# ClickHouse/libhdfs3

Hardware: AMD Instinct MI355X
Metric: device-resident CRC32C GiB/s over 512 B HDFS chunks; % of HBM roofline (higher is better)
Workload: dtype u8

## Files before the change

### libhdfs3_amd/csrc/crc32c_device.h

```cpp
#pragma once
#include <hip/hip_ext.h>

#include <type_traits>

#include "crc32c_kernels.h"
#include "crc32c_tables.h"

namespace hdfs3crc {
namespace {

constexpr int kCopies = 32;
constexpr int kLdsBytes = 128 * 1024;
constexpr int kLdsSlots = kLdsBytes / 16;

typedef uint32_t u32x4 __attribute__((ext_vector_type(4)));

constexpr int kFillPerThread = kLdsSlots / kBlockThreads;

__device__ __forceinline__ void fetch_tables(uint32_t (&v)[kFillPerThread],
                                             const uint32_t *__restrict__ g_tab) {
#pragma unroll
    for (int i = 0; i < kFillPerThread; ++i) {
        const int s = i * kBlockThreads + threadIdx.x;
        const int rowset = s >> 12, entry = (s >> 4) & 255, half = (s >> 3) & 1;
// ... 426 lines not shown
constexpr int kFoldLdsOff = kLdsBytes;
constexpr int kLdsBytesWave = kLdsBytes + 32 * 1024;

struct NibFold {
    const uint8_t *f;
    __device__ __forceinline__ explicit NibFold(const uint32_t *lds)
        : f(reinterpret_cast<const uint8_t *>(lds) + kFoldLdsOff + 4 * (threadIdx.x & 63)) {}
    __device__ __forceinline__ uint32_t ld(uint32_t off) const {
        return *reinterpret_cast<const uint32_t *>(f + off);
    }
    __device__ __forceinline__ uint32_t apply(uint32_t x) const {
        const uint32_t a0 = ld(((x << 8) & 0xF00u) + 0 * 4096);
        const uint32_t a1 = ld(((x << 4) & 0xF00u) + 1 * 4096);
        const uint32_t a2 = ld((x & 0xF00u) + 2 * 4096);
        const uint32_t a3 = ld(((x >> 4) & 0xF00u) + 3 * 4096);
        const uint32_t a4 = ld(((x >> 8) & 0xF00u) + 4 * 4096);
        const uint32_t a5 = ld(((x >> 12) & 0xF00u) + 5 * 4096);
        const uint32_t a6 = ld(((x >> 16) & 0xF00u) + 6 * 4096);
        const uint32_t a7 = ld(((x >> 20) & 0xF00u) + 7 * 4096);
        return xor3(xor3(a0, a1, a2), xor3(a3, a4, a5), a6 ^ a7);
    }
};

struct Look {
    uint32_t v[4];
};
__device__ __forceinline__ Look lookups(const Lut &t, uint32_t x) {
    Look l;
    l.v[0] = t.at<0>(3, x);
    l.v[1] = t.at<1>(2, x);
    l.v[2] = t.at<2>(1, x);
    l.v[3] = t.at<3>(0, x);
    return l;
}
__device__ __forceinline__ uint32_t combine(const Look &l, uint32_t next) {
    return xor3(xor3(l.v[0], l.v[1], l.v[2]), l.v[3], next);
}

constexpr int kHalfFoldOff = kLdsBytes;

template <int OFF = kHalfFoldOff>
__device__ __forceinline__ uint32_t fold_half(const uint8_t *lds, uint32_t x) {
    const uint32_t lo = x & 0x0F0F0F0Fu, hi = (x >> 4) & 0x0F0F0F0Fu;
    const uint32_t fb = (OFF & ~0xFFFF) + 4 * (threadIdx.x & 31);
    auto at = [&](uint32_t src, uint32_t byte, int off) {
        const uint32_t addr = __builtin_amdgcn_perm(src, fb, 0x0C020000u | ((4u + byte) << 8));
        return *reinterpret_cast<const uint32_t *>(lds + addr + (OFF & 0xFFFF) + off);
    };
    const uint32_t a0 = at(lo, 0, 0), a1 = at(hi, 0, 128), a2 = at(lo, 1, 4096), a3 = at(hi, 1, 4096 + 128);
    const uint32_t a4 = at(lo, 2, 8192), a5 = at(hi, 2, 8192 + 128), a6 = at(lo, 3, 12288);
    const uint32_t a7 = at(hi, 3, 12288 + 128);
    return xor3(xor3(a0, a1, a2), xor3(a3, a4, a5), a6 ^ a7);
}


struct SegLaunch {
    const DevSegment *seg;
    uint32_t nseg;
    uint64_t units;
    uint64_t uniform;
    unsigned long long *result;
    int check_short_tail;
    uint64_t stride;
    uint32_t kq, kr;
    uint8_t *dense_words;
    const uint32_t *unit_seg;
    DevSegment inl[kInlineSegments];
};

template <bool VERIFY>
__global__ __launch_bounds__(kBlockThreads) void crc32c_packets_kernel(
    const uint8_t *arena_c, uint8_t *arena_w, const DevPacket *__restrict__ pk,
    uint64_t n, uint32_t bpc, int check_short_tail, unsigned long long *result,
    const uint32_t *__restrict__ g_tab) {
    __shared__ __attribute__((aligned(16))) uint32_t lds[kLdsBytes / 4];
    fill_tables(lds, g_tab);
    lds_barrier();
    const Lut t(lds);
    const uint32_t lane = threadIdx.x & 63;
    const uint64_t waves = uint64_t(gridDim.x) * (kBlockThreads / 64);
    for (uint64_t w = uint64_t(blockIdx.x) * (kBlockThreads / 64) + (threadIdx.x >> 6); w < n;
         w += waves) {
        const DevPacket d = pk[w];
        const uint32_t chunks = (d.data_len + bpc - 1) / bpc;
        const uint8_t *data = arena_c + d.data_off;
        const bool al4 = (reinterpret_cast<uintptr_t>(arena_c + d.crc_off) & 3u) == 0;
        for (uint32_t k = lane; k < chunks; k += 64) {
            const uint32_t off = k * bpc;
            const uint32_t sz = d.data_len - off < bpc ? d.data_len - off : bpc;
            const uint32_t c = ~crc_run_any(t, 0xFFFFFFFFu, data + off, sz);
            if constexpr (VERIFY) {
                if ((sz == bpc || check_short_tail) &&
                    load_be32(arena_c + d.crc_off + 4ull * k, al4) != c)
                    atomicMax(result, ~((uint64_t(w) << 32) | k));
            } else {
                store_be32(arena_w + d.crc_off + 4ull * k, c, al4);
            }
        }
    }
}


#if HDFS3_LAB
__device__ unsigned long long *g_lab_clk = nullptr;
__device__ unsigned int g_lab_clk_cap = 0;
__device__ unsigned int g_lab_clk_n = 0;
// ... 143 lines not shown
```

### libhdfs3_amd/csrc/crc32c_experiments.hip

```cpp
#include "crc32c_wave.h"

namespace hdfs3crc {
namespace {

template <int BPC, bool V>
hipError_t launch_exp(const LaunchEnv &env, int variant, const ChunkLaunch &a) {
    const auto [tab, fold, grid_cap, s] = std::tie(env.tables, env.fold, env.grid_cap, env.stream);
    if constexpr (BPC > kRoundBytes) {
        if (variant == 115) return launch_r3<BPC, V, 1, true, true>(a, tab, fold, grid_cap, s);
        if (variant == 123) return launch_r3<BPC, V, 1, true>(a, tab, fold, grid_cap, s);
    }
    if constexpr (BPC <= kRoundBytes) {
        switch (variant) {
        case 92:
            return launch_wave3<BPC, V, false, true, kLabEarly>(a, tab, fold, grid_cap, s);
        case 93:
            return launch_wave3<BPC, V, false, false>(a, tab, fold, grid_cap, s);
        case 94:
            return launch_wave3<BPC, V, false, V>(a, tab, fold, grid_cap, s);
        case 95:
            return launch_wave3<BPC, V, false, true, kLabNoHold>(a, tab, fold, grid_cap, s);
        case 77:
            return launch_wave3<BPC, V, false, true, kLabNoMath>(a, tab, fold, grid_cap, s);
        case 99:
        case 100: {
            const uint64_t units = a.len / kRoundBytes;
            const uint64_t npk = variant == 99 ? 1 : 8;
            const uint64_t upp = units / npk;
            if (a.len % kRoundBytes || units % npk || (upp & (upp - 1)) || a.chunk_base) return hipErrorInvalidValue;
            ChunkLaunch p = a;
            p.npk = npk;
            p.pitch = upp * kRoundBytes;
            p.crc_pitch = upp * (kRoundBytes / BPC) * 4;
            p.last_len = uint32_t(upp * kRoundBytes);
            if (!packet_geom(p.pitch, p.last_len, npk, BPC, &p.geom)) return hipErrorInvalidValue;
            return launch_wave3<BPC, V, true, false>(p, tab, fold, grid_cap, s);
        }
        case 115:
            return launch_wave3<BPC, V, false, true, kLabPrio>(a, tab, fold, grid_cap, s);
        case 117:
            return launch_wave3<BPC, V, false, true, kLabNoPrio>(a, tab, fold, grid_cap, s);
        case 118:
            return launch_wave3<BPC, V, false, true, kLabNoStore>(a, tab, fold, grid_cap, s);
        case 119:
            return launch_wave3<BPC, V, false, true, kLabNearStore>(a, tab, fold, grid_cap, s);
        case 123:
            return launch_wave3<BPC, V, false, true>(a, tab, fold, grid_cap, s);
        case 122:
            return launch_wave3<BPC, V, false, true, kLabNoStage>(a, tab, fold, grid_cap, s);
        case 130:
            return launch_wave3<BPC, V, false, true, kLabStageWin>(a, tab, fold, grid_cap, s);
        case 157:
            return launch_wave3<BPC, V, false, true, kLabFull16>(a, tab, fold, grid_cap, s);
        case 128:
            return launch_wave3<BPC, V, false, true, kLabStorePlain>(a, tab, fold, grid_cap, s);
        case 146:
            return launch_wave3<BPC, V, false, true, kLabClock | kLabMid>(a, tab, fold, grid_cap, s);
        case 147:
            return launch_wave3<BPC, V, false, true, kLabNoTabLoad | kLabClock | kLabMid>(a, tab, fold, grid_cap, s);
        case 148:
            return launch_wave3<BPC, V, false, true, kLabNoTabLoad>(a, tab, fold, grid_cap, s);
        case 137:
            return launch_wave3<BPC, V, false, true, kLabWg1024>(a, tab, fold, grid_cap, s);
        case 162:
            return launch_wave3<BPC, V, false, true, kLabOneRound>(a, tab, fold, grid_cap, s);
        case 132:
            return launch_wave3<BPC, V, false, true, 0, 256>(a, tab, fold, grid_cap, s);
        case 134:
            return launch_wave3<BPC, V, false, true, 0, 512>(a, tab, fold, grid_cap, s);
        case 125:
            return launch_wave3<BPC, V, false, true, kLabClock>(a, tab, fold, grid_cap, s);
        case 78:
            return launch_wave3<BPC, V, false, true, kLabNoMath | kLabNoFill>(a, tab, fold, grid_cap, s);
        default: return hipErrorInvalidValue;
        }
    }
    return hipErrorInvalidValue;
}

}

hipError_t launch_experiment(const LaunchEnv &env, int variant, const ChunkLaunch &a, bool verify) {
    return dispatch_bpc<true>(a.bpc, [&](auto bpc) {
        return verify ? launch_exp<bpc(), true>(env, variant, a) : launch_exp<bpc(), false>(env, variant, a);
    });
}

void set_variant(int v) { g_variant = v; }

hipError_t lab_clock_buffer(unsigned long long *d, unsigned int cap, unsigned int *n_out) {
    unsigned int n = 0;
    hipError_t e = hipMemcpyFromSymbol(&n, HIP_SYMBOL(g_lab_clk_n), sizeof n);
    if (e != hipSuccess) return e;
    if (n_out) *n_out = n;
    const unsigned int zero = 0;
    if ((e = hipMemcpyToSymbol(HIP_SYMBOL(g_lab_clk), &d, sizeof d)) != hipSuccess) return e;
    if ((e = hipMemcpyToSymbol(HIP_SYMBOL(g_lab_clk_cap), &cap, sizeof cap)) != hipSuccess) return e;
    return hipMemcpyToSymbol(HIP_SYMBOL(g_lab_clk_n), &zero, sizeof zero);
}

hipError_t lab_wave_buffer(unsigned long long *d, unsigned int cap, unsigned int *n_out) {
    if (n_out) *n_out = g_lab_seq.exchange(0);
    hipError_t e;
    const unsigned long long *none = nullptr;
    if ((e = hipMemcpyToSymbol(HIP_SYMBOL(g_lab_wave), &none, sizeof none)) != hipSuccess) return e;
    if (!d || !cap) return hipSuccess;
// ... 47 lines not shown
```

### libhdfs3_amd/csrc/crc32c_kernels.hip

```cpp
#include "crc32c_wave.h"

namespace hdfs3crc {

#if HDFS3_LAB
int g_variant = 0;
#endif

namespace {

inline int clamped_grid(uint64_t want, uint64_t cap) { return int(want < cap ? want : cap); }

template <int BPC, bool V>
hipError_t launch_r(const LaunchEnv &env, const ChunkLaunch &a) {
#if HDFS3_LAB
    if (g_variant != 0) return launch_experiment(env, g_variant, a, V);
#endif
    if constexpr (BPC <= kRoundBytes)
        return launch_wave3<BPC, V, false, true>(a, env.tables, env.fold, env.grid_cap, env.stream);
    return launch_r3<BPC, V, 1, true>(a, env.tables, env.fold, env.grid_cap, env.stream);
}

template <int BPC, bool V>
hipError_t launch_p(const LaunchEnv &env, const ChunkLaunch &a) {
    const auto [tab, fold, grid_cap, s] = std::tie(env.tables, env.fold, env.grid_cap, env.stream);
#if HDFS3_LAB
    if (g_variant == 115) return launch_wave3<BPC, V, true, true, kLabPrio>(a, tab, fold, grid_cap, s);
    if (g_variant == 117) return launch_wave3<BPC, V, true, true, kLabNoPrio>(a, tab, fold, grid_cap, s);
    if (g_variant == 124) return launch_wave3<BPC, V, true, false>(a, tab, fold, grid_cap, s);
    if (g_variant == 132) return launch_wave3<BPC, V, true, true, 0, 256>(a, tab, fold, grid_cap, s);
    if (g_variant == 134) return launch_wave3<BPC, V, true, true, 0, 512>(a, tab, fold, grid_cap, s);
    if (g_variant == 137) return launch_wave3<BPC, V, true, true, kLabWg1024>(a, tab, fold, grid_cap, s);
    if (g_variant == 163) return launch_wave3<BPC, V, true, true, kLabNoHold>(a, tab, fold, grid_cap, s);
    if (g_variant == 162) return launch_wave3<BPC, V, true, true, kLabOneRound>(a, tab, fold, grid_cap, s);
#endif
    return launch_wave3<BPC, V, true, true>(a, tab, fold, grid_cap, s);
}

hipError_t launch_stream_kernel(const LaunchEnv &env, const ChunkLaunch &a, bool verify) {
    return dispatch_bpc(a.bpc, [&](auto bpc) {
        return verify ? launch_p<bpc(), true>(env, a) : launch_p<bpc(), false>(env, a);
    });
}

template <class... P, class... A>
hipError_t launch_vc(bool verify, void (*k_verify)(P...), void (*k_compute)(P...), int grid, int block,
                     hipStream_t stream, A... args) {
    hipLaunchKernelGGL(verify ? k_verify : k_compute, dim3(grid), dim3(block), 0, stream, args...);
    return hipGetLastError();
}

hipError_t grow_scratch(uint8_t **d, uint64_t *cap, hipEvent_t *used, uint64_t need) {
    if (need > *cap) {
        if (*used) {
            hipError_t e = hipEventSynchronize(*used);
            if (e != hipSuccess) return e;
        }
        if (*d) (void)hipFree(*d);
        *d = nullptr;
        *cap = 0;
        hipError_t e = hipMalloc(reinterpret_cast<void **>(d), need);
        if (e != hipSuccess) return e;
        *cap = need;
    }
    return *used ? hipSuccess : hipEventCreateWithFlags(used, hipEventDisableTiming);
}

__global__ __launch_bounds__(256) void crc32c_scatter_words_kernel(const uint8_t *__restrict__ src, uint8_t *dst,
                                                                   uint64_t src_pitch, uint64_t dst_pitch,
                                                                   uint64_t npk, uint32_t words, uint32_t last) {
    const uint64_t nwaves = uint64_t(gridDim.x) * 4;
    const uint32_t lane = threadIdx.x & 63;
    for (uint64_t p = uint64_t(blockIdx.x) * 4 + (threadIdx.x >> 6); p < npk; p += nwaves) {
        const uint32_t nw = (p + 1 == npk ? last : words) / 4;
        const uint32_t *s = reinterpret_cast<const uint32_t *>(src + p * src_pitch);
        uint32_t *d = reinterpret_cast<uint32_t *>(dst + p * dst_pitch);
        for (uint32_t i = lane; i < nw; i += 64) d[i] = s[i];
    }
}

}

void PieceScratch::release() {
    for (int i = 0; i < 2; ++i) {
        if (d[i]) (void)hipFree(d[i]);
        if (used[i]) (void)hipEventDestroy(used[i]);
// ... 142 lines not shown
        b.out_be = ws->d;
        b.crc_be = ws->d;
        b.crc_pitch = wpp;
        e = launch_stream_kernel(env, b, false);
        if (e != hipSuccess) return e;
        const int grid = clamped_grid((a.npk + 3) / 4, 1024);
        hipLaunchKernelGGL(crc32c_scatter_words_kernel, dim3(grid), dim3(256), 0, env.stream, ws->d, a.out_be, wpp,
                           cpitch, a.npk, uint32_t(wpp), uint32_t(last));
        e = hipGetLastError();
        if (e != hipSuccess) return e;
        return hipEventRecord(ws->used, env.stream);
    }
    return launch_stream_kernel(env, a, verify);
}

hipError_t launch_chunks(const LaunchEnv &env, const ChunkLaunch &a, bool verify) {
    const uint64_t chunks = (a.len + a.bpc - 1) / a.bpc;
    if (chunks == 0) return hipSuccess;
    const bool aligned = (reinterpret_cast<uintptr_t>(a.data) & 15u) == 0 &&
                         (reinterpret_cast<uintptr_t>(verify ? a.crc_be : a.out_be) & 3u) == 0;
    const uint64_t unit = a.bpc <= uint32_t(kRoundBytes) ? uint64_t(kRoundBytes) : a.bpc;
    const PieceScratch *pieces = env.pieces;
#if HDFS3_LAB
    if (g_variant == 123) pieces = nullptr;
#endif
    const bool multi_round = a.bpc == 8192 || a.bpc == 16384 || a.bpc == 65536;
    if (pieces && aligned && pieces_bpc(a.bpc) && a.len >= a.bpc && (!multi_round || a.len >= kPiecesMinBytes))
        return launch_pieces(env, a, verify);
    if (aligned && a.len >= unit && (round_bpc(a.bpc) || multi_round))
        return dispatch_bpc<true>(a.bpc, [&](auto bpc) {
            return verify ? launch_r<bpc(), true>(env, a) : launch_r<bpc(), false>(env, a);
        });
    const int grid = clamped_grid((chunks + kBlockThreads - 1) / kBlockThreads, uint64_t(env.grid_cap));
    return verify ? launch_t<0, true>(a, env.tables, grid, env.stream)
                  : launch_t<0, false>(a, env.tables, grid, env.stream);
}

hipError_t launch_packets(const LaunchEnv &env, const uint8_t *d_arena, const DevPacket *d_pk, uint64_t n,
                          uint32_t bpc, bool verify, int check_short_tail, unsigned long long *result) {
    if (n == 0) return hipSuccess;
    constexpr uint64_t kWaves = kBlockThreads / 64;
    return launch_vc(verify, crc32c_packets_kernel<true>, crc32c_packets_kernel<false>,
                     clamped_grid((n + kWaves - 1) / kWaves, uint64_t(env.grid_cap)), kBlockThreads, env.stream,
                     d_arena, verify ? nullptr : const_cast<uint8_t *>(d_arena), d_pk, n, bpc,
                     verify ? check_short_tail : 0, result, env.tables);
}

template <int BPC, bool V>
hipError_t launch_seg_t(const LaunchEnv &env, const SegLaunch &L) {
    const auto [tab, fold, grid_cap, s] = std::tie(env.tables, env.fold, env.grid_cap, env.stream);
#if HDFS3_LAB
    if (g_variant == 115) return launch_segments3<BPC, V, kLabPrio>(L, tab, fold, grid_cap, s);
    if (g_variant == 117) return launch_segments3<BPC, V, kLabNoPrio>(L, tab, fold, grid_cap, s);
    if (g_variant == 161) return launch_segments3<BPC, V, 0, 1024>(L, tab, fold, grid_cap, s);
#endif
    return launch_segments3<BPC, V>(L, tab, fold, grid_cap, s);
}

hipError_t launch_segments(const LaunchEnv &env, const DevSegment *d_seg, uint32_t nseg, uint64_t units,
                           uint64_t uniform, uint32_t bpc, bool verify, int check_short_tail,
                           unsigned long long *result, const DevSegment *h_inline, uint64_t stride,
                           uint8_t *dense_words, const uint32_t *unit_seg) {
    if (nseg == 0) return hipSuccess;
    SegLaunch L{};
    L.dense_words = dense_words;
    L.unit_seg = unit_seg;
    L.seg = d_seg;
    L.nseg = nseg;
    L.units = units;
    L.uniform = uniform;
    L.result = result;
    L.check_short_tail = check_short_tail;
    if (stride) {
        if (!h_inline || !uniform) return hipErrorInvalidValue;
        L.seg = nullptr;
        L.stride = stride;
        L.inl[0] = h_inline[0];
        L.inl[1] = h_inline[1];
    } else if (h_inline) {
        if (nseg > kInlineSegments) return hipErrorInvalidValue;
        L.seg = nullptr;
        for (uint32_t i = 0; i < nseg; ++i) L.inl[i] = h_inline[i];
    }
    return dispatch_bpc(bpc, [&](auto b) {
        return verify ? launch_seg_t<b(), true>(env, L) : launch_seg_t<b(), false>(env, L);
    });
}

namespace {

template <bool VERIFY>
__global__ __launch_bounds__(256) void crc32c_combine_segment_pieces_kernel(const DevSegment *__restrict__ seg,
                                                                            uint32_t n,
                                                                            const uint8_t *__restrict__ piece_be,
                                                                            uint32_t bpc,
                                                                            const uint32_t *__restrict__ g_fold,
                                                                            unsigned long long *result) {
    uint32_t col[32];
#pragma unroll
    for (int i = 0; i < 32; ++i) col[i] = g_fold[kFoldAdvance4096 + i];
    const uint32_t K = gf2_apply4(col, 0xFFFFFFFFu) ^ 0xFFFFFFFFu;
    const uint32_t R = bpc / kRoundBytes;
    const uint32_t lane = threadIdx.x & 63;
    const uint64_t nwaves = uint64_t(gridDim.x) * 4;
    for (uint64_t si = uint64_t(blockIdx.x) * 4 + (threadIdx.x >> 6); si < n; si += nwaves) {
        const DevSegment sd = seg[si];
// ... 169 lines not shown
```

### libhdfs3_amd/csrc/crc32c_tables.h

```cpp
#pragma once

#include <cstdint>

namespace hdfs3crc {

constexpr uint32_t kPolyReflected = 0x82F63B78u;
constexpr uint32_t kPolyCrc32 = 0xEDB88320u;
constexpr int kSlices = 4;
constexpr int kTableEntries = 256;
constexpr int kTableWords = kSlices * kTableEntries;

inline void build_slice_tables(uint32_t out[kSlices][kTableEntries], uint32_t poly = kPolyReflected) {
    for (uint32_t i = 0; i < 256; ++i) {
        uint32_t c = i;
        for (int k = 0; k < 8; ++k) c = (c >> 1) ^ ((c & 1u) ? poly : 0u);
        out[0][i] = c;
    }
    for (int k = 1; k < kSlices; ++k)
        for (int i = 0; i < 256; ++i)
            out[k][i] = out[0][out[k - 1][i] & 0xFFu] ^ (out[k - 1][i] >> 8);
}

inline uint32_t advance_bytes(const uint32_t t0[kTableEntries], uint32_t s, uint64_t n) {
    while (n--) s = t0[s & 0xFFu] ^ (s >> 8);
// ... 7 lines not shown
    return y;
}

inline void shift_cols(const uint32_t t0[kTableEntries], uint64_t n, uint32_t cols[32]) {
    for (int i = 0; i < 32; ++i) cols[i] = advance_bytes(t0, 1u << i, n);
}

constexpr int kFoldGs[4] = {8, 16, 32, 64};
constexpr int kFoldOffset[4] = {0, 8, 24, 56};
constexpr int kFoldAdvance4096 = 120 * 32;
constexpr int kFoldWords = kFoldAdvance4096 + 32;

inline int fold_set_index(int g) { return g == 8 ? 0 : g == 16 ? 1 : g == 32 ? 2 : 3; }

inline void build_fold_matrices(const uint32_t t0[kTableEntries], uint32_t out[kFoldWords]) {
    uint32_t f64[32];
    shift_cols(t0, 64, f64);
    for (int s = 0; s < 4; ++s) {
        const int g = kFoldGs[s];
        uint32_t m[32];
        for (int i = 0; i < 32; ++i) m[i] = 1u << i;
        for (int j = g - 1; j >= 0; --j) {
            for (int i = 0; i < 32; ++i) out[(kFoldOffset[s] + j) * 32 + i] = m[i];
            for (int i = 0; i < 32; ++i) m[i] = apply_cols(f64, m[i]);
        }
    }
    shift_cols(t0, 4096, out + kFoldAdvance4096);
}

constexpr int kFoldNibbleWords = 8 * 16 * 64;

inline void build_fold_nibbles(const uint32_t fold[kFoldWords], int set, uint32_t out[kFoldNibbleWords]) {
    const int g = kFoldGs[set];
    for (int lane = 0; lane < 64; ++lane) {
        const uint32_t *cols = fold + (kFoldOffset[set] + lane % g) * 32;
        for (int k = 0; k < 8; ++k)
            for (uint32_t e = 0; e < 16; ++e)
                out[(k * 16 + e) * 64 + lane] = apply_cols(cols, e << (4 * k));
    }
}

inline void build_fold_nibbles_pre(const uint32_t t0[kTableEntries], const uint32_t fold[kFoldWords], int set,
                                   uint32_t out[kFoldNibbleWords]) {
    const int g = kFoldGs[set];
    for (int lane = 0; lane < 64; ++lane) {
        const uint32_t *cols = fold + (kFoldOffset[set] + lane % g) * 32;
        for (int k = 0; k < 8; ++k)
            for (uint32_t e = 0; e < 16; ++e)
                out[(k * 16 + e) * 64 + lane] = apply_cols(cols, advance_bytes(t0, e << (4 * k), 4));
    }
}

constexpr int kFoldAffineOff = kFoldWords;
constexpr int kFoldAffineOldOff = kFoldAffineOff + 4 * kFoldNibbleWords;
constexpr int kFoldImageWords = kFoldAffineOldOff + 4 * kFoldNibbleWords;
inline void build_fold_affine(const uint32_t t0[kTableEntries], int set, uint32_t out[kFoldNibbleWords]) {
    const int g = kFoldGs[set];
    const uint32_t kc = advance_bytes(t0, 0xFFFFFFFFu, uint64_t(64) * g) ^ 0xFFFFFFFFu;
    for (int lane = 0; lane < 64; ++lane)
        if (lane % g == g - 1)
            for (uint32_t e = 0; e < 16; ++e) out[e * 64 + lane] ^= kc;
    for (int i = 0; i < kFoldNibbleWords; ++i) out[i] = __builtin_bswap32(out[i]);
}

}
```

### libhdfs3_amd/csrc/crc32c_wave.h

```cpp
#pragma once

#include "crc32c_device.h"

namespace hdfs3crc {
namespace {

constexpr int kLabEarly = 1;
constexpr int kLabNoMath = 2;
constexpr int kLabNoHold = 4;
constexpr int kLabNoFill = 8;
constexpr int kLabPrio = 16;
constexpr int kLabNoPrio = 32;
constexpr int kLabNoStore = 64;
constexpr int kLabNearStore = 128;
constexpr int kLabNoStage = 1024;
constexpr int kLabStageWin = 2048;
constexpr int kLabClock = 4096;
constexpr int kLabStorePlain = 8192;
constexpr int kLabWg1024 = 16384;
constexpr int kLabNoTabLoad = 2097152;
constexpr int kLabFull16 = 8388608;
constexpr int kLabOneRound = 4194304;
constexpr int kLabMid = 1048576;
constexpr int kStageWords = 512;
constexpr uint32_t kStageMaxRounds(int bpc) { return uint32_t(bpc / 16); }

constexpr uint32_t kPrioMinRounds = 16;

typedef __attribute__((address_space(1))) const uint32_t gcu32;
typedef __attribute__((address_space(1))) const uint8_t gcu8;
typedef __attribute__((address_space(1))) uint8_t gu8;
typedef __attribute__((address_space(1))) uint32_t gu32;
typedef __attribute__((address_space(1))) unsigned long long gu64;
typedef __attribute__((address_space(4))) const SegLaunch CSegLaunch;
typedef __attribute__((address_space(4))) const DevSegment CDevSegment;

struct WView {
    const uint8_t *p;
    uint8_t *w;
    uint64_t key;
    uint32_t nb;
};

template <int CPU>
struct BlockWalk {
    static constexpr bool kLaneView = true;
    static constexpr bool kContiguous = true;
    const uint8_t *data;
    uint8_t *words;
    uint64_t key0, first, stride;
    uint32_t K;
    const uint8_t *dummy;
    uint32_t kq = 0, kr = 0;
    __device__ __forceinline__ WView view(uint32_t k) const {
        const uint64_t u = first + uint64_t(k) * stride;
        const bool in = k < K;
        return WView{in ? data + u * kRoundBytes : dummy, in ? words + 4 * CPU * u : const_cast<uint8_t *>(dummy),
                     key0 + CPU * u, uint32_t(kRoundBytes)};
    }
};

template <int CPU>
struct PitchWalk {
    static constexpr bool kLaneView = true;
    static constexpr bool kContiguous = false;
    const uint8_t *data;
    uint8_t *words;
    uint64_t dpitch, wpitch, first, stride;
    uint32_t K;
    uint32_t upp, magic, shift, ptail, lunits, ltail, lpk;
    const uint8_t *dummy;
    __device__ __forceinline__ WView view(uint32_t k) const {
        const uint32_t u = uint32_t(first + uint64_t(k) * stride);
        const uint32_t pk = uint32_t((uint64_t(u) * magic) >> shift), r = u - pk * upp;
        const bool lastp = pk == lpk;
        const uint32_t nb = r + 1 == (lastp ? lunits : upp) ? (lastp ? ltail : ptail) : uint32_t(kRoundBytes);
        const bool in = k < K;
        return WView{in ? data + uint64_t(pk) * dpitch + uint64_t(r) * kRoundBytes : dummy,
// ... 35 lines not shown
            }
            return lo;
        }
    }
    __device__ __forceinline__ WView view(uint32_t k) {
        if (k >= K) return WView{dummy, const_cast<uint8_t *>(dummy), 0, uint32_t(kRoundBytes)};
        const uint64_t u = first + uint64_t(k) * stride;
        if (u < c_begin || u >= c_end) {
            uint32_t si;
            if constexpr (UNI) {
                si = seg_of(u);
            } else {
                const uint32_t nx = c_si + 1;
                if (nx < L->nseg && u >= rfl64(segp(nx)->unit_begin) &&
                    u < rfl64(segp(nx)->unit_begin) + units(rfl64(segp(nx)->len)))
                    si = nx;
                else if (L->unit_seg)
                    si = __builtin_amdgcn_readfirstlane(
                        ((__attribute__((address_space(4))) const uint32_t *)(L->unit_seg))[u]);
                else
                    si = seg_of(u);
            }
            if (L->stride) {
                const bool lastp = si + 1 >= L->nseg;
                c_begin = uint64_t(si) * L->uniform;
                c_wlen = wlen(lastp ? L->inl[1].len : L->inl[0].len);
                c_end = c_begin + (lastp ? units(L->inl[1].len) : L->uniform);
                c_data = L->inl[0].data + uint64_t(si) * L->stride;
                c_crc = L->dense_words ? L->dense_words + 4 * CPU * c_begin : L->inl[0].crc + uint64_t(si) * L->stride;
                c_key = uint64_t(si) << 32;
            } else {
                CDevSegment *sd = segp(si);
                c_begin = rfl64(sd->unit_begin);
                c_wlen = wlen(rfl64(sd->len));
                c_end = c_begin + (c_wlen + kRoundBytes - 1) / kRoundBytes;
                c_data = reinterpret_cast<const uint8_t *>(rfl64(reinterpret_cast<uint64_t>(sd->data)));
                c_crc = L->dense_words ? L->dense_words + 4 * CPU * c_begin
                                       : reinterpret_cast<uint8_t *>(rfl64(reinterpret_cast<uint64_t>(sd->crc)));
                c_key = rfl64(sd->key_base);
            }
            c_si = si;
        }
        const uint64_t r = u - c_begin, left = c_wlen - r * kRoundBytes;
        return WView{c_data + r * kRoundBytes, c_crc + 4 * CPU * r, c_key + CPU * r,
                     left < kRoundBytes ? uint32_t(left) : uint32_t(kRoundBytes)};
    }
};

template <int BPC, bool VERIFY, bool SOLO, bool HOLD, int LAB, int TPB, class Walk>
__device__ __forceinline__ void wave_rounds(Walk &walk, uint32_t *lds, const uint32_t *__restrict__ g_tab,
                                            const uint32_t *__restrict__ g_nib, unsigned long long *result,
                                            unsigned long long *lab_mid = nullptr) {
    constexpr int G = BPC / 64;
    constexpr bool kHalfFold = G <= 32;
    constexpr bool LATE = (LAB & kLabEarly) == 0, NOMATH = (LAB & kLabNoMath) != 0;
    constexpr bool kWrong = (LAB & (kLabNoMath | kLabNoFill | kLabNoTabLoad)) != 0;
    const uint32_t lane = threadIdx.x & 63;
    const uint32_t j = lane % G;
    const uint32_t lane_off = 64 * (lane & 15) + 16 * (lane >> 4);
    const uint32_t K = walk.K;

    constexpr int kFillIters = 1024 / TPB;
    static_assert(kFillIters * TPB == 1024, "TPB divides 1024");
    uint32_t tw[kFillIters];
    u32x4 n0[kFillIters], n1[kFillIters];
#pragma unroll
    for (int f = 0; f < kFillIters; ++f) {
        const uint32_t t = threadIdx.x + f * TPB;
        if constexpr ((LAB & kLabNoTabLoad) != 0) {
            tw[f] = t * 0x9E3779B9u;
            n0[f] = u32x4{t, t ^ 1u, t ^ 2u, t ^ 3u};
            n1[f] = n0[f];
            continue;
        }
        tw[f] = g_tab[t];
        if constexpr (kHalfFold) {
            const uint32_t fk = 2 * (t >> 8) + ((t >> 3) & 1), fe = (t >> 4) & 15, fc = 4 * (t & 7);
            n0[f] = *reinterpret_cast<const u32x4 *>(g_nib + (fk * 16 + fe) * 64 + fc);
        } else {
            n0[f] = *reinterpret_cast<const u32x4 *>(g_nib + 8 * t);
            n1[f] = *reinterpret_cast<const u32x4 *>(g_nib + 8 * t + 4);
        }
    }
    WView cv0 = walk.view(0), cv1 = walk.view(1);
    __builtin_amdgcn_sched_barrier(0);
    Round a0, a1, b0, b1;
    load_round_buf<true>(a0, cv0.p, lane_off, cv0.nb);
    load_round_buf<true>(a1, cv1.p, lane_off, cv1.nb);
    __builtin_amdgcn_sched_barrier(0);
#pragma unroll
    for (int f = 0; f < kFillIters; ++f) {
        const uint32_t tt = threadIdx.x + f * TPB, slice = tt >> 8, entry = tt & 255;
        const uint32_t slot0 = ((slice >> 1) << 16 | entry << 8 | (slice & 1) << 7) / 16;
        const uint32_t w = tw[f];
        const uint32_t byte_t = (slot0 | (tt & 7)) << 4;
#pragma unroll
        for (int r = 0; r < ((LAB & kLabNoFill) ? 0 : 8); ++r)
            *reinterpret_cast<u32x4 *>(reinterpret_cast<uint8_t *>(lds) + (byte_t ^ uint32_t(16 * r))) = u32x4{w, w, w, w};
        if constexpr (kHalfFold) {
            reinterpret_cast<u32x4 *>(lds + kHalfFoldOff / 4)[tt] = n0[f];
        } else {
            u32x4 *dst = reinterpret_cast<u32x4 *>(reinterpret_cast<uint8_t *>(lds) + kFoldLdsOff) + 2 * tt;
            dst[0] = n0[f];
            dst[1] = n1[f];
        }
    }
    lds_barrier();
    if constexpr ((LAB & kLabMid) != 0) lab_mid[0] = __builtin_amdgcn_s_memrealtime();
    const Lut t(lds);
    const NibFold nf(lds);
    auto fold = [&](uint32_t x) -> uint32_t {
        if constexpr (kHalfFold) return fold_half(reinterpret_cast<const uint8_t *>(lds), x);
        return nf.apply(x);
    };
    const uint32_t woff = 4 * (lane / G);
    const uint32_t coff = (lane / G) * BPC;
    WView pv0 = walk.view(2), pv1 = walk.view(3);

    auto wrsrc = [](const WView &v) {
        return __builtin_amdgcn_make_buffer_rsrc(v.w, 0, __builtin_amdgcn_readfirstlane(v.nb / (BPC / 4)), 0x00020000);
    };
    auto want_of = [&](const WView &v) -> uint32_t {
        if constexpr (VERIFY) return __builtin_amdgcn_raw_buffer_load_b32(wrsrc(v), woff, 0, 0);
        return 0;
    };
    constexpr bool kHold = HOLD && !VERIFY && G == 8;
    constexpr bool kAddr = !Walk::kLaneView;
    auto held_store = [&](gu8 *p, uint32_t v) { *(gu32 *)p = v; };
    uint32_t line = 0;
    uint32_t hold[kHold ? 8 : 1];
    gu32 *laddr = nullptr;
    gu32 *hold_addr[kHold && kAddr ? 8 : 1];
    uint32_t nheld = 0, hold_base = 0;
    auto flush = [&]() {
#pragma unroll
        for (int i = 0; i < (kHold ? 8 : 0); ++i) {
            if (uint32_t(i) < nheld && ((LAB & kLabNoStore) == 0 || hold[i] == 0x9E3779B9u)) {
                if constexpr ((LAB & kLabNearStore) != 0 && !kAddr) {
                    *(gu32 *)((gu8 *)walk.view(0).w + 4 * lane) = hold[i];
                } else if constexpr (kAddr) {
                    if (hold_addr[i]) *hold_addr[i] = hold[i];
                } else {
                    const uint32_t kk = 8 * (hold_base + nheld - 1 - i) + (lane >> 3);
                    if (kk < K) {
                        const WView v = walk.view(kk);
                        if ((lane & 7) * BPC < v.nb) held_store((gu8 *)v.w + 4 * (lane & 7), hold[i]);
                    }
                }
            }
        }
        hold_base += nheld;
        nheld = 0;
    };
    constexpr bool kStage = !VERIFY && (LAB & kStageWords) != 0 && Walk::kContiguous && kHalfFold && TPB == 1024;
    constexpr uint32_t kCpw = 64 / G;
    constexpr uint32_t kSR = kStageMaxRounds(BPC);
    uint32_t *stage = lds + kLdsBytesWave / 4 - 4096;
    const uint32_t slot = threadIdx.x >> 6;
    auto stage_store = [&](gu8 *p, uint32_t v) {
        if constexpr ((LAB & kLabNoStore) != 0) {
            if (v != 0x9E3779B9u) return;
        }
        if constexpr (kStage && (LAB & kLabStorePlain) == 0) {
            const uint64_t wb = rfl64(reinterpret_cast<uint64_t>(walk.words));
// ... 298 lines not shown
        if constexpr ((LAB & kLabMid) != 0)
            clk.end(a.lab_seq, ((lab_mid[0] - clk.r0) & 0x1FFFFF) | ((lab_mid[1] - clk.r0) & 0x1FFFFF) << 21 |
                                   ((lab_mid[2] - clk.r0) & 0x1FFFFF) << 42);
        else
            clk.end(a.lab_seq);
    }
#endif
}

template <int BPC, bool VERIFY, bool UNI, int LAB = 0, int TPB = kBlockThreads>
__global__ __launch_bounds__(TPB) void crc32c_segments_kernel(SegLaunch L, const uint32_t *__restrict__ g_tab,
                                                              const uint32_t *__restrict__ g_nib) {
    static_assert(BPC <= kRoundBytes && BPC % 512 == 0, "one-round units");
    __shared__ __attribute__((aligned(16))) uint32_t lds[kLdsBytesWave / 4];
    constexpr int kCpu = kRoundBytes / BPC;
    constexpr int kWpb = TPB / 64;
    const uint64_t nwaves = uint64_t(gridDim.x) * kWpb;
    const uint64_t wave = uint64_t(blockIdx.x) * kWpb + __builtin_amdgcn_readfirstlane(threadIdx.x >> 6);
    SegWalk<kCpu, UNI> w{(CSegLaunch *)(&L), wave, nwaves, L.kq + (wave < L.kr ? 1u : 0u),
                         reinterpret_cast<const uint8_t *>(g_tab)};
    wave_rounds<BPC, VERIFY, false, !VERIFY && BPC == 512, LAB, TPB>(w, lds, g_tab, g_nib, L.result);

    if (L.dense_words) return;
    const Lut t(lds);
    for (uint64_t si = uint64_t(threadIdx.x) * gridDim.x + blockIdx.x; si < L.nseg;
         si += uint64_t(gridDim.x) * TPB) {
        DevSegment sd;
        if (L.stride) {
            sd = L.inl[0];
            sd.data += si * L.stride;
            sd.crc += si * L.stride;
            sd.len = si + 1 < L.nseg ? L.inl[0].len : L.inl[1].len;
            sd.key_base = si << 32;
        } else {
            sd = L.seg ? L.seg[si] : L.inl[si];
        }
        if (sd.len % BPC) {
            const uint64_t c = sd.len / BPC;
            const uint32_t v = ~crc_run_lines(t, 0xFFFFFFFFu, sd.data + c * BPC, uint32_t(sd.len % BPC));
            if constexpr (VERIFY) {
                if (L.check_short_tail && load_be32(sd.crc + 4 * c, true) != v)
                    atomicMax(L.result, ~(unsigned long long)(sd.key_base + c));
            } else {
                store_be32(sd.crc + 4 * c, v, true);
            }
        }
    }
}

constexpr uint64_t kSoloTailMaxBytes = uint64_t(256) << 20;

template <int BPC, bool V, bool PITCH, bool SOLO, int LAB = 0, int TPB = kBlockThreads>
hipError_t launch_wave3(const ChunkLaunch &a, const uint32_t *tab, const uint32_t *fold, int grid_cap, hipStream_t s) {
    constexpr int G = BPC / 64;
    constexpr int set = G == 8 ? 0 : G == 16 ? 1 : G == 32 ? 2 : 3;
    const uint32_t *nib = fold + ((LAB & kLabFull16) ? kFoldAffineOldOff : kFoldAffineOff) + set * kFoldNibbleWords;
    const uint64_t units = PITCH ? (a.npk - 1) * a.geom.upp + a.geom.lunits : a.len / kRoundBytes;
    const uint64_t rpw = (LAB & kLabOneRound) != 0 && units <= 4096 ? 1 : 2;
    const uint64_t need = (units + rpw * (TPB / 64) - 1) / (rpw * (TPB / 64));
    int grid = int(need < uint64_t(grid_cap) ? need : uint64_t(grid_cap));
    if (grid < 1) grid = 1;
    const uint64_t nwaves = uint64_t(grid) * (TPB / 64);
    if (units / nwaves >= (uint64_t(1) << 32)) return hipErrorInvalidValue;
    ChunkLaunch b = a;
    if constexpr ((LAB & kLabClock) != 0) b.lab_seq = g_lab_seq++;
    b.kq = uint32_t(units / nwaves);
    b.kr = uint32_t(units % nwaves);
    if constexpr ((V || PITCH) && TPB == 1024 && (LAB & kLabWg1024) == 0) {
        constexpr int kSmall = (!V && PITCH) ? kLabNoHold : 0;
        if (units <= 4096) return launch_wave3<BPC, V, PITCH, SOLO, LAB | kSmall, 256>(a, tab, fold, grid_cap, s);
        if (units <= 16384) return launch_wave3<BPC, V, PITCH, SOLO, LAB, 512>(a, tab, fold, grid_cap, s);
    }
    if constexpr (!V && BPC <= 2048 && !PITCH && TPB == 1024 &&
                  (LAB & (kStageWords | kLabNoStage | kLabNoHold)) == 0) {
        const bool words_fit = units * uint64_t(4 * (kRoundBytes / BPC)) < (uint64_t(1) << 31);
        if (words_fit && (b.kq + (b.kr ? 1u : 0u) <= kStageMaxRounds(BPC) || BPC != 512 || (LAB & kLabStageWin) != 0))
            return launch_wave3<BPC, V, PITCH, SOLO, LAB | kStageWords, TPB>(a, tab, fold, grid_cap, s);
    }
    if (a.overlap_previous) {
        if constexpr (SOLO) {
            if (units * kRoundBytes <= kSoloTailMaxBytes) {
                hipExtLaunchKernelGGL((crc32c_wave_kernel<BPC, V, PITCH, true, LAB, TPB>), dim3(grid),
                                      dim3(TPB), 0, s, nullptr, nullptr, hipExtAnyOrderLaunch, b, tab, nib);
                return hipGetLastError();
            }
        }
        hipExtLaunchKernelGGL((crc32c_wave_kernel<BPC, V, PITCH, false, LAB, TPB>), dim3(grid),
                              dim3(TPB), 0, s, nullptr, nullptr, hipExtAnyOrderLaunch, b, tab, nib);
    } else {
        hipLaunchKernelGGL((crc32c_wave_kernel<BPC, V, PITCH, false, LAB, TPB>), dim3(grid), dim3(TPB),
                           0, s, b, tab, nib);
    }
    return hipGetLastError();
}

template <int BPC, bool V, int LAB = 0, int TPB = kBlockThreads>
hipError_t launch_segments3(const SegLaunch &in, const uint32_t *tab, const uint32_t *fold, int grid_cap,
                            hipStream_t s) {
    if constexpr (TPB == 1024) {
        if (in.units <= 4096) return launch_segments3<BPC, V, LAB, 256>(in, tab, fold, grid_cap, s);
        if (in.units <= 16384) return launch_segments3<BPC, V, LAB, 512>(in, tab, fold, grid_cap, s);
    }
    constexpr int G = BPC / 64;
    constexpr int set = G == 8 ? 0 : G == 16 ? 1 : G == 32 ? 2 : 3;
    constexpr uint64_t kWpb = TPB / 64;
    const uint32_t *nib = fold + ((LAB & kLabFull16) ? kFoldAffineOldOff : kFoldAffineOff) + set * kFoldNibbleWords;
    SegLaunch L = in;
    const uint64_t need = (L.units + 2 * kWpb - 1) / (2 * kWpb);
    const uint64_t tail_need = (L.nseg + TPB - 1) / TPB;
    uint64_t g = need > tail_need ? need : tail_need;
    g = g < uint64_t(grid_cap) ? g : uint64_t(grid_cap);
    const int grid = int(g > 0 ? g : 1);
    const uint64_t nwaves = uint64_t(grid) * kWpb;
    if (L.units / nwaves >= (uint64_t(1) << 32)) return hipErrorInvalidValue;
    L.kq = uint32_t(L.units / nwaves);
    L.kr = uint32_t(L.units % nwaves);
    if (L.uniform)
        hipLaunchKernelGGL((crc32c_segments_kernel<BPC, V, true, LAB, TPB>), dim3(grid), dim3(TPB), 0, s, L, tab, nib);
    else
        hipLaunchKernelGGL((crc32c_segments_kernel<BPC, V, false, LAB, TPB>), dim3(grid), dim3(TPB), 0, s, L, tab, nib);
    return hipGetLastError();
}

}
}
```

### libhdfs3_amd/csrc/hdfs3_crc.cpp

```cpp
#include "hdfs3_crc.h"
#include "md5.h"

#include <hip/hip_runtime.h>

#include <algorithm>
#include <cerrno>
#include <cstddef>
#include <cstdarg>
#include <cstdio>
#include <cstdlib>
#include <cstring>
#include <vector>
#include <mutex>
#include <new>

#include "copy_pool.h"
#include "crc32c_kernels.h"
#include "crc32c_tables.h"
#include "crc_compose.h"
#include "ctx.h"
#include "numa.h"

namespace hdfs3crc {
uint32_t host_update(uint32_t state, const void *p, size_t n);
}

using namespace hdfs3crc;

namespace hdfs3crc {

thread_local char g_err[512] = "";

int fail(int code, const char *fmt, ...) {
    va_list ap;
    va_start(ap, fmt);
    vsnprintf(g_err, sizeof(g_err), fmt, ap);
    va_end(ap);
    return code;
}

}

namespace hdfs3crc {

#if HDFS3_LAB
constexpr size_t kFoldUploadBytes = sizeof(uint32_t) * kFoldImageWords;
#else
constexpr size_t kFoldUploadBytes = sizeof(uint32_t) * kFoldAffineOldOff;
#endif

struct HostImage {
    uint32_t t[kSlices][kTableEntries];
    uint32_t fold[kFoldImageWords];
};

const HostImage *host_images() {
    static HostImage img[2];
    static std::once_flag once;
    std::call_once(once, [] {
        const uint32_t polys[2] = {kPolyReflected, kPolyCrc32};
        for (int p = 0; p < 2; ++p) {
            build_slice_tables(img[p].t, polys[p]);
            build_fold_matrices(img[p].t[0], img[p].fold);
            for (int set = 0; set < 4; ++set) {
                uint32_t *nib = img[p].fold + kFoldAffineOff + set * kFoldNibbleWords;
                build_fold_nibbles_pre(img[p].t[0], img[p].fold, set, nib);
                build_fold_affine(img[p].t[0], set, nib);
#if HDFS3_LAB
                uint32_t *old = img[p].fold + kFoldAffineOldOff + set * kFoldNibbleWords;
                build_fold_nibbles(img[p].fold, set, old);
                build_fold_affine(img[p].t[0], set, old);
#endif
            }
        }
    });
    return img;
}

}

namespace {

int hip_fail(hipError_t e, const char *what) {
    const int code = e == hipErrorOutOfMemory ? -ENOMEM
                     : e == hipErrorInvalidValue ? -EINVAL
                     : e == hipErrorNoDevice || e == hipErrorInvalidDevice ? -ENODEV
                                                                           : -EIO;
    return fail(code, "%s: %s", what, hipGetErrorString(e));
}

#define HIP_TRY(expr)                                  \
    do {                                               \
        hipError_t e_ = (expr);                        \
        if (e_ != hipSuccess) return hip_fail(e_, #expr); \
    } while (0)

}

namespace {

int check_args(hdfs3_crc_ctx *ctx, uint32_t bpc) {
    if (!ctx) return fail(-EINVAL, "null hdfs3_crc_ctx");
    if (bpc == 0) return fail(-EINVAL, "bytes per checksum must be positive");
    return 0;
}

int grow_slot(Slot &s, size_t data_bytes, size_t crc_bytes) {
    if (data_bytes > s.data_cap) {
        if (s.h_data) (void)hipHostFree(s.h_data);
        if (s.d_data) (void)hipFree(s.d_data);
        s.h_data = s.d_data = nullptr;
        s.data_cap = 0;
        HIP_TRY(hipHostMalloc(reinterpret_cast<void **>(&s.h_data), data_bytes, pinned_host_flags()));
        HIP_TRY(hipMalloc(reinterpret_cast<void **>(&s.d_data), data_bytes));
        s.data_cap = data_bytes;
    }
    if (crc_bytes > s.crc_cap) {
        if (s.h_crc) (void)hipHostFree(s.h_crc);
        if (s.d_crc) (void)hipFree(s.d_crc);
        s.h_crc = s.d_crc = nullptr;
        s.crc_cap = 0;
        HIP_TRY(hipHostMalloc(reinterpret_cast<void **>(&s.h_crc), crc_bytes, pinned_host_flags()));
        HIP_TRY(hipMalloc(reinterpret_cast<void **>(&s.d_crc), crc_bytes));
        s.crc_cap = crc_bytes;
    }
    return 0;
// ... 1170 lines not shown
```

Before: 6007.

## Use byte-indexed fold tables for verify path at 512-byte chunks

Adds a byte-granular fold table (256 entries by 32 lanes) built on the host, and uses it in the wave kernel's fold step when verifying 512-byte chunks. The old path did eight nibble-indexed LDS lookups; the new one does four byte-indexed lookups with per-lane rotation to spread LDS bank access. This halves the LDS reads and XORs in the fold but doubles the fold table staged into LDS. The previous nibble fold stays reachable as lab variant 164.

Result: no change. 6005, median of 2 (-0.0%).

```diff
diff --git a/libhdfs3_amd/csrc/crc32c_device.h b/libhdfs3_amd/csrc/crc32c_device.h
--- a/libhdfs3_amd/csrc/crc32c_device.h
+++ b/libhdfs3_amd/csrc/crc32c_device.h
@@ -502,6 +502,29 @@
     const uint32_t a7 = at(hi, 3, 12288 + 128);
     return xor3(xor3(a0, a1, a2), xor3(a3, a4, a5), a6 ^ a7);
 }
+
+struct ByteFold {
+    uint32_t base[4];
+    uint32_t rot;
+    __device__ __forceinline__ ByteFold() {
+        const uint32_t j = threadIdx.x & 7, v = (threadIdx.x >> 3) & 3;
+#pragma unroll
+        for (uint32_t i = 0; i < 4; ++i) {
+            base[i] = uint32_t(kHalfFoldOff) + 4 * (8 * ((i + v) & 3) + j);
+            asm("" : "+v"(base[i]));
+        }
+        rot = (8 * v + 25) & 31;
+    }
+    __device__ __forceinline__ uint32_t apply(const uint8_t *lds, uint32_t x) const {
+        const uint32_t r = __builtin_amdgcn_alignbit(x, x, rot);
+        auto at = [&](uint32_t s, int i) {
+            return *reinterpret_cast<const uint32_t *>(lds + ((s & 0x7F80u) | base[i]));
+        };
+        const uint32_t a0 = at(r, 0), a1 = at(r >> 8, 1), a2 = at(r >> 16, 2);
+        const uint32_t a3 = at(__builtin_amdgcn_alignbit(r, r, 24), 3);
+        return xor3(a0, a1, a2) ^ a3;
+    }
+};
 
 
 struct SegLaunch {
diff --git a/libhdfs3_amd/csrc/crc32c_experiments.hip b/libhdfs3_amd/csrc/crc32c_experiments.hip
--- a/libhdfs3_amd/csrc/crc32c_experiments.hip
+++ b/libhdfs3_amd/csrc/crc32c_experiments.hip
@@ -52,6 +52,8 @@
             return launch_wave3<BPC, V, false, true, kLabStageWin>(a, tab, fold, grid_cap, s);
         case 157:
             return launch_wave3<BPC, V, false, true, kLabFull16>(a, tab, fold, grid_cap, s);
+        case 164:
+            return launch_wave3<BPC, V, false, true, kLabNibFold>(a, tab, fold, grid_cap, s);
         case 128:
             return launch_wave3<BPC, V, false, true, kLabStorePlain>(a, tab, fold, grid_cap, s);
         case 146:
diff --git a/libhdfs3_amd/csrc/crc32c_kernels.hip b/libhdfs3_amd/csrc/crc32c_kernels.hip
--- a/libhdfs3_amd/csrc/crc32c_kernels.hip
+++ b/libhdfs3_amd/csrc/crc32c_kernels.hip
@@ -31,6 +31,7 @@
     if (g_variant == 134) return launch_wave3<BPC, V, true, true, 0, 512>(a, tab, fold, grid_cap, s);
     if (g_variant == 137) return launch_wave3<BPC, V, true, true, kLabWg1024>(a, tab, fold, grid_cap, s);
     if (g_variant == 163) return launch_wave3<BPC, V, true, true, kLabNoHold>(a, tab, fold, grid_cap, s);
+    if (g_variant == 164) return launch_wave3<BPC, V, true, true, kLabNibFold>(a, tab, fold, grid_cap, s);
     if (g_variant == 162) return launch_wave3<BPC, V, true, true, kLabOneRound>(a, tab, fold, grid_cap, s);
 #endif
     return launch_wave3<BPC, V, true, true>(a, tab, fold, grid_cap, s);
@@ -279,6 +280,7 @@
 #if HDFS3_LAB
     if (g_variant == 115) return launch_segments3<BPC, V, kLabPrio>(L, tab, fold, grid_cap, s);
     if (g_variant == 117) return launch_segments3<BPC, V, kLabNoPrio>(L, tab, fold, grid_cap, s);
+    if (g_variant == 164) return launch_segments3<BPC, V, kLabNibFold>(L, tab, fold, grid_cap, s);
     if (g_variant == 161) return launch_segments3<BPC, V, 0, 1024>(L, tab, fold, grid_cap, s);
 #endif
     return launch_segments3<BPC, V>(L, tab, fold, grid_cap, s);
diff --git a/libhdfs3_amd/csrc/crc32c_tables.h b/libhdfs3_amd/csrc/crc32c_tables.h
--- a/libhdfs3_amd/csrc/crc32c_tables.h
+++ b/libhdfs3_amd/csrc/crc32c_tables.h
@@ -83,7 +83,9 @@
 }
 
 constexpr int kFoldAffineOff = kFoldWords;
-constexpr int kFoldAffineOldOff = kFoldAffineOff + 4 * kFoldNibbleWords;
+constexpr int kFoldByteWords = 256 * 32;
+constexpr int kFoldByteOff = kFoldAffineOff + 4 * kFoldNibbleWords;
+constexpr int kFoldAffineOldOff = kFoldByteOff + kFoldByteWords;
 constexpr int kFoldImageWords = kFoldAffineOldOff + 4 * kFoldNibbleWords;
 inline void build_fold_affine(const uint32_t t0[kTableEntries], int set, uint32_t out[kFoldNibbleWords]) {
     const int g = kFoldGs[set];
@@ -94,4 +96,26 @@
     for (int i = 0; i < kFoldNibbleWords; ++i) out[i] = __builtin_bswap32(out[i]);
 }
 
+inline void build_fold_bytes(const uint32_t t0[kTableEntries], const uint32_t fold[kFoldWords],
+                             uint32_t out[kFoldByteWords]) {
+    constexpr int set = 0, g = 8;
+    const uint32_t kc = advance_bytes(t0, 0xFFFFFFFFu, uint64_t(64) * g) ^ 0xFFFFFFFFu;
+    for (int j = 0; j < g; ++j) {
+        const uint32_t *cols = fold + (kFoldOffset[set] + j) * 32;
+        for (int tau = 0; tau < 4; ++tau)
+            for (uint32_t e = 0; e < 256; ++e) {
+                const uint32_t m = apply_cols(cols, advance_bytes(t0, e << (8 * tau), 4));
+                out[e * 32 + 8 * tau + j] = __builtin_bswap32(m ^ (j == g - 1 && tau == 0 ? kc : 0u));
+            }
+    }
 }
+
+inline uint32_t apply_fold_bytes(const uint32_t img[kFoldByteWords], int lane, uint32_t x) {
+    const int j = lane & 7, v = (lane >> 3) & 3;
+    const uint32_t xr = v ? (x >> (8 * v)) | (x << (32 - 8 * v)) : x;
+    uint32_t y = 0;
+    for (int i = 0; i < 4; ++i) y ^= img[((xr >> (8 * i)) & 0xFFu) * 32 + 8 * ((i + v) & 3) + j];
+    return y;
+}
+
+}
diff --git a/libhdfs3_amd/csrc/crc32c_wave.h b/libhdfs3_amd/csrc/crc32c_wave.h
--- a/libhdfs3_amd/csrc/crc32c_wave.h
+++ b/libhdfs3_amd/csrc/crc32c_wave.h
@@ -17,6 +17,7 @@
 constexpr int kLabStageWin = 2048;
 constexpr int kLabClock = 4096;
 constexpr int kLabStorePlain = 8192;
+constexpr int kLabNibFold = 32768;
 constexpr int kLabWg1024 = 16384;
 constexpr int kLabNoTabLoad = 2097152;
 constexpr int kLabFull16 = 8388608;
@@ -24,6 +25,17 @@
 constexpr int kLabMid = 1048576;
 constexpr int kStageWords = 512;
 constexpr uint32_t kStageMaxRounds(int bpc) { return uint32_t(bpc / 16); }
+
+constexpr bool byte_fold(int bpc, bool verify, int lab) {
+    return verify && bpc == 512 && (lab & (kLabNibFold | kLabFull16)) == 0;
+}
+template <int BPC, bool V, int LAB>
+inline const uint32_t *fold_image(const uint32_t *fold) {
+    constexpr int G = BPC / 64;
+    constexpr int set = G == 8 ? 0 : G == 16 ? 1 : G == 32 ? 2 : 3;
+    if constexpr (byte_fold(BPC, V, LAB)) return fold + kFoldByteOff;
+    return fold + ((LAB & kLabFull16) ? kFoldAffineOldOff : kFoldAffineOff) + set * kFoldNibbleWords;
+}
 
 constexpr uint32_t kPrioMinRounds = 16;
 
@@ -165,7 +177,8 @@
                                             const uint32_t *__restrict__ g_nib, unsigned long long *result,
                                             unsigned long long *lab_mid = nullptr) {
     constexpr int G = BPC / 64;
-    constexpr bool kHalfFold = G <= 32;
+    constexpr bool kByteFold = byte_fold(BPC, VERIFY, LAB);
+    constexpr bool kHalfFold = G <= 32 && !kByteFold;
     constexpr bool LATE = (LAB & kLabEarly) == 0, NOMATH = (LAB & kLabNoMath) != 0;
     constexpr bool kWrong = (LAB & (kLabNoMath | kLabNoFill | kLabNoTabLoad)) != 0;
     const uint32_t lane = threadIdx.x & 63;
@@ -190,6 +203,9 @@
         if constexpr (kHalfFold) {
             const uint32_t fk = 2 * (t >> 8) + ((t >> 3) & 1), fe = (t >> 4) & 15, fc = 4 * (t & 7);
             n0[f] = *reinterpret_cast<const u32x4 *>(g_nib + (fk * 16 + fe) * 64 + fc);
+        } else if constexpr (kByteFold) {
+            n0[f] = *reinterpret_cast<const u32x4 *>(g_nib + 4 * t);
+            n1[f] = *reinterpret_cast<const u32x4 *>(g_nib + 4 * (t + 1024));
         } else {
             n0[f] = *reinterpret_cast<const u32x4 *>(g_nib + 8 * t);
             n1[f] = *reinterpret_cast<const u32x4 *>(g_nib + 8 * t + 4);
@@ -212,6 +228,9 @@
             *reinterpret_cast<u32x4 *>(reinterpret_cast<uint8_t *>(lds) + (byte_t ^ uint32_t(16 * r))) = u32x4{w, w, w, w};
         if constexpr (kHalfFold) {
             reinterpret_cast<u32x4 *>(lds + kHalfFoldOff / 4)[tt] = n0[f];
+        } else if constexpr (kByteFold) {
+            reinterpret_cast<u32x4 *>(lds + kHalfFoldOff / 4)[tt] = n0[f];
+            reinterpret_cast<u32x4 *>(lds + kHalfFoldOff / 4)[tt + 1024] = n1[f];
         } else {
             u32x4 *dst = reinterpret_cast<u32x4 *>(reinterpret_cast<uint8_t *>(lds) + kFoldLdsOff) + 2 * tt;
             dst[0] = n0[f];
@@ -222,7 +241,9 @@
     if constexpr ((LAB & kLabMid) != 0) lab_mid[0] = __builtin_amdgcn_s_memrealtime();
     const Lut t(lds);
     const NibFold nf(lds);
+    const ByteFold bf;
     auto fold = [&](uint32_t x) -> uint32_t {
+        if constexpr (kByteFold) return bf.apply(reinterpret_cast<const uint8_t *>(lds), x);
         if constexpr (kHalfFold) return fold_half(reinterpret_cast<const uint8_t *>(lds), x);
         return nf.apply(x);
     };
@@ -627,9 +648,7 @@
 
 template <int BPC, bool V, bool PITCH, bool SOLO, int LAB = 0, int TPB = kBlockThreads>
 hipError_t launch_wave3(const ChunkLaunch &a, const uint32_t *tab, const uint32_t *fold, int grid_cap, hipStream_t s) {
-    constexpr int G = BPC / 64;
-    constexpr int set = G == 8 ? 0 : G == 16 ? 1 : G == 32 ? 2 : 3;
-    const uint32_t *nib = fold + ((LAB & kLabFull16) ? kFoldAffineOldOff : kFoldAffineOff) + set * kFoldNibbleWords;
+    const uint32_t *nib = fold_image<BPC, V, LAB>(fold);
     const uint64_t units = PITCH ? (a.npk - 1) * a.geom.upp + a.geom.lunits : a.len / kRoundBytes;
     const uint64_t rpw = (LAB & kLabOneRound) != 0 && units <= 4096 ? 1 : 2;
     const uint64_t need = (units + rpw * (TPB / 64) - 1) / (rpw * (TPB / 64));
@@ -676,10 +695,8 @@
         if (in.units <= 4096) return launch_segments3<BPC, V, LAB, 256>(in, tab, fold, grid_cap, s);
         if (in.units <= 16384) return launch_segments3<BPC, V, LAB, 512>(in, tab, fold, grid_cap, s);
     }
-    constexpr int G = BPC / 64;
-    constexpr int set = G == 8 ? 0 : G == 16 ? 1 : G == 32 ? 2 : 3;
     constexpr uint64_t kWpb = TPB / 64;
-    const uint32_t *nib = fold + ((LAB & kLabFull16) ? kFoldAffineOldOff : kFoldAffineOff) + set * kFoldNibbleWords;
+    const uint32_t *nib = fold_image<BPC, V, LAB>(fold);
     SegLaunch L = in;
     const uint64_t need = (L.units + 2 * kWpb - 1) / (2 * kWpb);
     const uint64_t tail_need = (L.nseg + TPB - 1) / TPB;
diff --git a/libhdfs3_amd/csrc/hdfs3_crc.cpp b/libhdfs3_amd/csrc/hdfs3_crc.cpp
--- a/libhdfs3_amd/csrc/hdfs3_crc.cpp
+++ b/libhdfs3_amd/csrc/hdfs3_crc.cpp
@@ -72,6 +72,7 @@
                 build_fold_affine(img[p].t[0], set, old);
 #endif
             }
+            build_fold_bytes(img[p].t[0], img[p].fold, img[p].fold + kFoldByteOff);
         }
     });
     return img;
```
